# TUM-PIK-ESM/Terrarium.jl

Measured on AMD Instinct MI355X. Metric: column-steps/sec, higher is better.
Workload: dtype f64

## Files before the change

### terrarium.jl_amd/csrc/terrarium_hip.hip

```cpp
#include "trm_host.hpp"

#include <dlfcn.h>

using namespace trm;
using namespace trmh;

namespace {
thread_local std::string g_create_error;
}

namespace trmh {
int fail(trm_ctx* ctx, int code, const std::string& msg) {
    if (ctx) ctx->err = msg;
    else g_create_error = msg;
    return code;
}
}

namespace {

template <class NF> struct HostGrid {
    std::vector<NF> zF, zC, dzc, rdzc, rdzf, dzf, psiz;
    NF dzf_bot, dzf_top;
    void build(int Nz, const double* thickness) {
        std::vector<double> cs(Nz);
        double acc = thickness[0];
        cs[0] = acc;
        for (int n = 1; n < Nz; ++n) { acc = acc + thickness[n]; cs[n] = acc; }
        zF.resize(Nz + 1);
        for (int f = 0; f < Nz; ++f) zF[f] = (NF)(-cs[Nz - 1 - f]);
        zF[Nz] = NF(0);
        NF Fm1 = zF[0] - (zF[1] - zF[0]);
        NF Fp1 = zF[Nz] + (zF[Nz] - zF[Nz - 1]);
        zC.resize(Nz);
        dzc.resize(Nz);
        rdzc.resize(Nz);
        for (int k = 0; k < Nz; ++k) {
            zC[k] = (zF[k + 1] + zF[k]) / NF(2);
            dzc[k] = zF[k + 1] - zF[k];
            rdzc[k] = NF(1) / dzc[k];
        }
        NF Cm1 = (zF[0] + Fm1) / NF(2);
        NF Cp1 = (Fp1 + zF[Nz]) / NF(2);
        dzf.resize(Nz + 1);
        rdzf.resize(Nz + 1);
        for (int f = 0; f <= Nz; ++f) {
            NF hi = (f < Nz) ? zC[f] : Cp1;
            NF lo = (f > 0) ? zC[f - 1] : Cm1;
            dzf[f] = hi - lo;
            rdzf[f] = NF(1) / dzf[f];
        }
        dzf_bot = dzf[0];
        dzf_top = dzf[Nz];
        psiz.resize(Nz);
        for (int k = 0; k < Nz; ++k) psiz[k] = zC[k] - zF[Nz];
    }
};

template <class NF> DevParams<NF> make_dev_params(const trm_params& q) {
    DevParams<NF> p;
    NF rho_soc = (NF)q.rho_soc, rho_org = (NF)q.rho_org, por_m = (NF)q.por_mineral, por_o = (NF)q.por_organic;
    p.org = rho_soc / ((NF(1) - por_o) * rho_org);
    p.por = (NF(1) - p.org) * por_m + p.org * por_o;
    p.rpor = NF(1) / p.por;
    p.solid_frac = NF(1) - p.por;
    p.frac_organic = p.solid_frac * p.org;
    p.frac_mineral = p.solid_frac * (NF(1) - p.org);
    p.sk_water = std::sqrt((NF)q.k_water);
    p.sk_ice = std::sqrt((NF)q.k_ice);
    p.sk_air = std::sqrt((NF)q.k_air);
    p.kterm_mineral = std::sqrt((NF)q.k_mineral) * p.frac_mineral;
    p.kterm_organic = std::sqrt((NF)q.k_organic) * p.frac_organic;
    p.c_water = (NF)q.c_water;
    p.c_ice = (NF)q.c_ice;
    p.c_air = (NF)q.c_air;
    p.cterm_mineral = (NF)q.c_mineral * p.frac_mineral;
    p.cterm_organic = (NF)q.c_organic * p.frac_organic;
    p.L = (NF)q.rho_w * (NF)q.Lsl;
    p.K_sat = (NF)q.K_sat;
    p.theta_res = (NF)q.theta_res;
// ... 74 lines not shown
    v.lwu = F(TRM_FIELD_SURFACE_LONGWAVE_UP);
    v.rnet = F(TRM_FIELD_SURFACE_NET_RADIATION);
    v.Hs = F(TRM_FIELD_SENSIBLE_HEAT_FLUX);
    v.Hl = F(TRM_FIELD_LATENT_HEAT_FLUX);
    v.evap = F(TRM_FIELD_EVAPORATION_GROUND);
    v.infil = F(TRM_FIELD_INFILTRATION);
    v.runoff = F(TRM_FIELD_SURFACE_RUNOFF);
    v.Tair = F(TRM_FIELD_AIR_TEMPERATURE);
    v.pres = F(TRM_FIELD_AIR_PRESSURE);
    v.wind = F(TRM_FIELD_WINDSPEED);
    v.qair = F(TRM_FIELD_SPECIFIC_HUMIDITY);
    v.rain = F(TRM_FIELD_RAINFALL);
    v.swd = F(TRM_FIELD_SURFACE_SHORTWAVE_DOWN);
    v.lwd = F(TRM_FIELD_SURFACE_LONGWAVE_DOWN);
    v.albedo = F(TRM_FIELD_ALBEDO);
    v.emissivity = F(TRM_FIELD_EMISSIVITY);
    v.zC = (const NF*)c->d_zC;
    v.zF = (const NF*)c->d_zF;
    v.dzc = (const NF*)c->d_dzc;
    v.rdzc = (const NF*)c->d_rdzc;
    v.rdzf = (const NF*)c->d_rdzf;
    v.psiz = (const NF*)c->d_psiz;
    v.lvl = (const NF*)c->d_lvl;
    v.Fvwc = c->opt_vwc_field ? (const NF*)((&s == &c->stage && c->stage_vwc_own) ? c->stage.f[TRM_FIELD_VWC_FORCING] : c->state.f[TRM_FIELD_VWC_FORCING]) : nullptr;
    BcGeom<NF>& g = v.g;
    g.dzf_bot = (NF)c->dzf_bot;
    g.dzf_top = (NF)c->dzf_top;
    g.hdzf_bot = g.dzf_bot / NF(2);
    g.hdzf_top = g.dzf_top / NF(2);
    g.rhdzf_bot = NF(1) / g.hdzf_bot;
    g.rhdzf_top = NF(1) / g.hdzf_top;
    g.Az = (NF)c->Az;
    g.V_bot = g.Az * (NF)c->dzc_bot;
    g.V_top = g.Az * (NF)c->dzc_top;
    g.rV_bot = NF(1) / g.V_bot;
    g.rV_top = NF(1) / g.V_top;
    g.zF_top = (NF)c->h_zF[c->Nz];
    g.dzc_top = (NF)c->dzc_top;
    v.status = c->d_status;
    for (int a = 0; a < TRM_BCV_COUNT; ++a)
        for (int b = 0; b < 2; ++b) {
            v.bc.kind[a][b] = c->bc_kind[a][b];
            void* val = (&s == &c->stage && c->bc_value_stage[a][b]) ? c->bc_value_stage[a][b] : c->bc_value[a][b];
            v.bc.value[a][b] = val ? val : c->d_zero;
        }
    fill_small_table(v);
    return v;
}

template <class NF> View<NF> sub_view(const View<NF>& v, long lo, long n) {
    View<NF> s = v;
    s.Nh = n;
    const long c3 = lo * v.Nzp;
    auto p3 = [&](NF*& q) { if (q) q += c3; };
    auto p2 = [&](NF*& q) { if (q) q += lo; };
    auto c2 = [&](const NF*& q) { if (q) q += lo; };
    p3(s.U); p3(s.sat); p3(s.T); p3(s.liq); p3(s.psi); p3(s.Kf); p3(s.G_U); p3(s.G_sat);
    if (s.Fvwc) s.Fvwc += c3;
    p2(s.S); p2(s.wt); p2(s.Kf_top); p2(s.G_S);
    p2(s.Ts); p2(s.ghf); p2(s.infil); p2(s.swu); p2(s.lwu); p2(s.rnet); p2(s.Hs); p2(s.Hl); p2(s.evap); p2(s.runoff);
    p2(s.top_T); p2(s.top_sat); p2(s.top_liq);
// ... 563 lines not shown
        TRM_HIP(c, hipMemsetAsync(s.kf_top, 0, (size_t)c->Nh * c->esize, c->stream));
    }
    TRM_HIP(c, hipStreamSynchronize(c->stream));
    return TRM_OK;
}

template <class NF> int upload_grid(trm_ctx* c, const double* thickness) {
    HostGrid<NF> g;
    g.build(c->Nz, thickness);
    auto up = [&](void** d, const std::vector<NF>& h) -> int {
        TRM_HIP(c, hipMalloc(d, h.size() * sizeof(NF)));
        TRM_HIP(c, hipMemcpyAsync(*d, h.data(), h.size() * sizeof(NF), hipMemcpyHostToDevice, c->stream));
    TRM_HIP(c, hipStreamSynchronize(c->stream));
        return TRM_OK;
    };
    int rc;
    if ((rc = up(&c->d_zC, g.zC))) return rc;
    if ((rc = up(&c->d_zF, g.zF))) return rc;
    if ((rc = up(&c->d_dzc, g.dzc))) return rc;
    if ((rc = up(&c->d_rdzc, g.rdzc))) return rc;
    if ((rc = up(&c->d_rdzf, g.rdzf))) return rc;
    if ((rc = up(&c->d_psiz, g.psiz))) return rc;
    {
        std::vector<NF> lvl((size_t)c->Nz * 8, NF(0));
        for (int k = 0; k < c->Nz; ++k) {
            NF* q = &lvl[(size_t)k * 8];
            q[0] = g.zC[k]; q[1] = g.psiz[k]; q[2] = g.zF[k]; q[3] = g.dzc[k]; q[4] = g.rdzc[k]; q[5] = g.rdzf[k]; q[6] = g.rdzf[k + 1];
        }
        if ((rc = up(&c->d_lvl, lvl))) return rc;
    }
    c->h_zF.assign(g.zF.begin(), g.zF.end());
    c->h_zC.assign(g.zC.begin(), g.zC.end());
    c->h_dzc.assign(g.dzc.begin(), g.dzc.end());
    c->h_dzf.assign(g.dzf.begin(), g.dzf.end());
    c->dzf_bot = g.dzf_bot;
    c->dzf_top = g.dzf_top;
    c->dzc_bot = g.dzc[0];
    c->dzc_top = g.dzc[c->Nz - 1];
    return TRM_OK;
}

template <class NF> int fill_row(trm_ctx* c, int field, double value) {
    std::vector<NF> h((size_t)c->Nh, (NF)value);
    TRM_HIP(c, hipMemcpyAsync(c->state.f[field], h.data(), h.size() * sizeof(NF), hipMemcpyHostToDevice, c->stream));
    TRM_HIP(c, hipStreamSynchronize(c->stream));
    return TRM_OK;
}

__host__ __device__ inline double nan_min(double a, double b) { return (a != a || b != b) ? (a + b) : (a < b ? a : b); }
__host__ __device__ inline double nan_max(double a, double b) { return (a != a || b != b) ? (a + b) : (a > b ? a : b); }
template <class NF, int OP> __global__ void k_reduce_rows(const NF* f3, const NF* ftop, long Nh, int Nzp, int Nz, int is3d,
                                                          const NF* weight, double* partial) {
// ... 418 lines not shown

int trm_destroy(trm_ctx* c) {
    if (!c) return TRM_OK;
    (void)hipSetDevice(c->device);
    (void)trm_comm_destroy(c);
    if (c->own_stream) (void)hipStreamSynchronize(c->own_stream);
    for (int f = 0; f < TRM_FIELD_COUNT; ++f) {
        if (c->state.f[f]) (void)hipFree(c->state.raw[f]);
        if (c->stage.f[f]) (void)hipFree(c->stage.raw[f]);
        if (c->saved.f[f]) (void)hipFree(c->saved.raw[f]);
    }
    if (c->d_gran) (void)hipFree(c->d_gran);
    if (c->state.kf_top) (void)hipFree(c->state.kf_top);
    if (c->stage.kf_top) (void)hipFree(c->stage.kf_top);
    if (c->saved.kf_top) (void)hipFree(c->saved.kf_top);
    for (int a = 0; a < TRM_BCV_COUNT; ++a)
        for (int b = 0; b < 2; ++b)
        {
            if (c->bc_value[a][b]) (void)hipFree(c->bc_value[a][b]);
            if (c->bc_value_stage[a][b]) (void)hipFree(c->bc_value_stage[a][b]);
        }
    for (auto& sr : c->series)
        if (sr.d_values) (void)hipFree(sr.d_values);
    for (void* q : {c->d_zC, c->d_zF, c->d_dzc, c->d_rdzc, c->d_rdzf, c->d_psiz, c->d_lvl, c->d_rootf, c->d_zero, c->d_top3, (void*)c->d_status, (void*)c->d_reduce, c->d_io, c->d_series_table, c->d_series_rows})
        if (q) (void)hipFree(q);
    if (c->ev0) (void)hipEventDestroy(c->ev0);
    if (c->ev1) (void)hipEventDestroy(c->ev1);
    if (c->copy_stream) { (void)hipStreamSynchronize(c->copy_stream); (void)hipStreamDestroy(c->copy_stream); }
    if (c->copy_done) (void)hipEventDestroy(c->copy_done);
    if (c->copy_order) (void)hipEventDestroy(c->copy_order);
    if (c->h_stage) (void)hipHostFree(c->h_stage);
    for (auto& st : c->row_stage) {
        if (st.pending) (void)hipEventSynchronize(st.done);
        if (st.done) (void)hipEventDestroy(st.done);
        if (st.h) (void)hipHostFree(st.h);
    }
    for (void* q : {(void*)c->d_ring_inv, (void*)c->d_ring_idx, c->d_ring})
        if (q) (void)hipFree(q);
    for (auto& a : c->averages)
        if (a.d_sum) (void)hipFree(a.d_sum);
    for (double* q : c->d_acc_partial)
        if (q) (void)hipFree(q);
    release_tangent(c);
    release_adjoint(c);

    if (c->own_stream) (void)hipStreamDestroy(c->own_stream);
    if (c->args && c->args_free) c->args_free(c->args);
// ... 1261 lines not shown
```

### terrarium.jl_amd/csrc/trm_column.hpp

```cpp
#pragma once
#include "trm_kernels.hpp"
#include "trm_average.hpp"
#include <cstddef>
#include <type_traits>

namespace trm {

enum { PROG_EULER = 0, PROG_HEUN = 1, PROG_MULTI = 2 };
enum { PSI_STORED = 0, PSI_LAST = 1, PSI_INTERIOR = 2 };
#ifndef TRM_FRONT_DIAG
#define TRM_FRONT_DIAG 0
#endif
#ifndef TRM_FRONT_POLL_SLEEP
#define TRM_FRONT_POLL_SLEEP 4
#endif
#ifndef TRM_FRONT_PRIO
#define TRM_FRONT_PRIO 3
#endif

template <class NF> struct Cell { NF U, sat, T, liq, psi; };
struct LaneInfo { int lane, k; bool is_bot, is_top, act; unsigned long long m_act, m_bot, m_top; };
template <class NF> struct ColumnBC {
    NF bTb, bTt;
    NF flux_U, flux_S;
// ... 69 lines not shown
        const NF Kc_m = shfl_up1<NF, LPC>(Kc);
        const NF Kmin = jl_min(Kc, Kc_m);
        t.Kf_lo = BCSIG >= 0 ? mask_pick(m_bot | m_top, Kc, Kmin) : ((is_bot || is_top) ? Kc : Kmin);
    }
    if (RICHARDS) {
        const NF Kf_lo = t.Kf_lo;
        const NF Kf_up = shfl_up1<NF, LPC>(Kf_lo), Kf_dn = shfl_dn1<NF, LPC>(Kf_lo), psi_sh = shfl_up1<NF, LPC>(c.psi);
        const NF Kf_m = Kf_up;
        const NF Kf_p = at_top(Kc, Kf_dn);
        const NF psi_m = at_bot(c.psi, psi_sh);
        const NF g_lo = (c.psi - psi_m) * L.rdzf_lo;
        const NF Ks_lo = upwind_conductivity(g_lo, Kf_m, Kf_lo, Kf_p);
        const NF qW_lo = -Ks_lo * g_lo;
        const NF qW_sh = shfl_dn1<NF, LPC>(qW_lo);
        const NF zero_or_nan = c.psi - c.psi;
        const NF qW_t = -jl_min(Kc, NF(0)) * zero_or_nan;
        const NF qW_hi = at_top(qW_t, qW_sh);
        const NF dtheta = -((qW_hi - qW_lo) * L.rdzc) + NF(0) + p.vwc_forcing;
        t.gS = NF(0) + div_const_nsz(dtheta, p.por, p.rpor);
    }
    return t;
}

template <class NF, bool RICHARDS, int LPC>
TRM_DEV NF column_advance(const View<NF>& v, const LevelGeom<NF>& L, const LaneInfo& ln, int Nz, const ColumnBC<NF>& bc,
                          NF U0, NF sat0, NF& gU, NF& gS, NF dt, Cell<NF>& n, NF& z0, bool& bad) {
    if (bc.has_U) gU += bc.flux_U;
    n.U = U0 + gU * dt;
    if (!RICHARDS) bad = bad || (ln.act && is_nan(n.U));
    n.sat = sat0;
    z0 = NF(0);
    NF over = NF(0);
    if (RICHARDS) {
        if (bc.has_S) gS += bc.flux_S;
        NF snew = sat0 + gS * dt;
        bad = bad || (ln.act && __builtin_isunordered(n.U, snew));
        over = repair_saturation<NF, LPC>(v, snew, ln.k, Nz, ln.m_act, ln.is_bot, ln.is_top, L, ln.m_bot, ln.m_top);
        z0 = water_table<NF, LPC>(snew, ln.m_act, ln.lane, L);
        n.sat = snew;
    }
    return over;
}

template <class NF, bool RICHARDS, int HYD>
TRM_DEV Frac<NF> column_closure(const DevParams<NF>& p, const LevelGeom<NF>& L, NF z0, Cell<NF>& n, uint32_t& viol) {
    const Frac<NF> f = energy_closure_wave<NF, RICHARDS ? 2 : 1>(p, n.U, n.sat, n.liq, n.T, viol);
    n.psi = RICHARDS ? pressure_head<NF, HYD, true>(p, n.sat, L.zC, L.psiz, z0) : NF(0);
    return f;
}

template <class NF> struct SurfaceRegs {
    SebIn<NF> in;
    SebOut<NF> out;
};

enum { SLOT_T_BOT = 0, SLOT_T_TOP, SLOT_FU_BOT, SLOT_FU_TOP, SLOT_FS_BOT, SLOT_FS_TOP, SLOT_TAIR, SLOT_PRES, SLOT_WIND, SLOT_QAIR,
       SLOT_RAIN, SLOT_SWD, SLOT_LWD, SLOT_ALBEDO, SLOT_EMISSIVITY, SLOT_COUNT };
template <class NF> struct SeriesTable {
    const NF* base[SLOT_COUNT];
    NF* dst[SLOT_COUNT];
// ... 104 lines not shown
    const int finalize = a.finalize, write_kf = a.write_kf;
    const bool need_kc = RICHARDS || write_kf;
    const int i = wave * CPW + sub;
    const bool colok = i < Nh;
    ln.act = colok && ln.k < Nz;
    ln.m_act = wave_ballot(colok) & wave_ballot(ln.k < Nz);
    const int ii = colok ? i : Nh - 1;
    const int col_first = __builtin_amdgcn_readfirstlane(wave * CPW);
#endif
    const unsigned ib0 = (unsigned)ii * (unsigned)sizeof(NF);
    const unsigned cb0 = ((unsigned)ii * (unsigned)v.Nzp + (unsigned)(ln.k < Nz ? ln.k : Nz - 1)) * (unsigned)sizeof(NF);
    uint32_t viol = 0;
    bool bad = false;

    TRM_PHASE("loads+derive");
    Cell<NF> c;
    c.U = ldg(v.U, cb0);
    c.sat = ldg(v.sat, cb0);
    static_assert(DERIVE == DERIVE_NONE || DERIVE == DERIVE_T_LIQ, "the column program reads T / liq or derives both (the liquid fraction alone and the "
                  "pressure head as well were measured and lost: EXPERIMENTS.md; their instances were removed in round 5)");
    constexpr bool DERIVE_TL = DERIVE == DERIVE_T_LIQ;
    c.psi = (RICHARDS && !PSI_IN) ? ldg(v.psi, cb0) : NF(0);
    if (!DERIVE_TL) { c.T = ldg(v.T, cb0); c.liq = ldg(v.liq, cb0); }
    const LevelGeom<NF> L = level_geom(v, ln.k);
    constexpr bool SIG = BCSIG >= 0;
    const bool seb = SIG ? (BCSIG & BCSIG_LAND) != 0 : p.seb != 0;
    const bool vTb = SIG ? (BCSIG & BCSIG_T_BOT) != 0 : v.bc.kind[2][0] == 1, vTt = SIG ? (BCSIG & BCSIG_T_TOP) != 0 : v.bc.kind[2][1] == 1;
    const bool bU = SIG ? (BCSIG & BCSIG_FU_BOT) != 0 : v.bc.kind[0][0] == 2, bS = RICHARDS && (SIG ? (BCSIG & BCSIG_FS_BOT) != 0 : v.bc.kind[1][0] == 2);
    const bool tU = !SEB_INLINE && (seb || (SIG ? (BCSIG & BCSIG_FU_TOP) != 0 : v.bc.kind[0][1] == 2));
    const bool tS = RICHARDS && !SEB_INLINE && (seb || (SIG ? (BCSIG & BCSIG_FS_TOP) != 0 : v.bc.kind[1][1] == 2));
    const unsigned jo0 = (unsigned)(col_first < Nh ? col_first : Nh - 1) * (unsigned)sizeof(NF), jo1 = (unsigned)(col_first + 1 < Nh ? col_first + 1 : Nh - 1) * (unsigned)sizeof(NF);
    struct ColVal { NF x0, x1; };
    constexpr bool DEFER = SCALAR_IN && CPW == 2 && BCSIG >= 0;
    auto col_req = [&](const NF* ptr) -> ColVal {
        if (!SCALAR_IN) return ColVal{ldg(ptr, ib0), NF(0)};
        const NF x0 = sld_off<NF>(ptr, jo0);
        if (CPW == 1) return ColVal{x0, NF(0)};
        const NF x1 = sld_off<NF>(ptr, jo1);
        if (DEFER) return ColVal{x0, x1};
        return ColVal{upper ? x1 : x0, NF(0)};
    };
    auto pick_column = [&](NF x0, NF x1) -> NF {
#if TRM_PICK_EXEC
        if (__builtin_constant_p(x0 == x1) && x0 == x1) return x0;
        if constexpr (sizeof(NF) == 8) {
            NF r;
            unsigned long long save;
// ... 133 lines not shown
            bc.flux_S = ln.is_top ? eS_t : NF(0);
            TRM_PHASE("rare-");
        }
    };
    Cell<NF> n = c;
    Tendency<NF> t{};
    NF gU_out = NF(0), gS_out = NF(0), GS_out = NF(0), z0 = NF(0);

    NF over = NF(0), over_stage = NF(0);
    Frac<NF> f_new{};
    double accU = 0.0, accSat = 0.0, accT = 0.0, accLiq = 0.0, accPsi = 0.0, acc2 = 0.0;
    auto acc_top = [&](unsigned am, double w, int slot, NF x) {
        if (am & (1u << slot)) {
            const NF xt = shfl_from<NF, LPC>(x, Nz - 1);
            if (ln.k == slot - ACC_S) acc2 = acc2 + w * (double)xt;
        }
    };
    if (PROG == PROG_HEUN) {
        t = column_tendencies<NF, RICHARDS, HYD, LPC, BCSIG>(v, p, L, ln, c, bc.bTb, bc.bTt, need_kc, viol, DERIVE_TL ? &f_in : nullptr);
        const NF G1U = t.gU, G1S = t.gS;
        NF gU = G1U, gS = G1S, z0s;
        Cell<NF> s;
        front_wait();
        over_stage = column_advance<NF, RICHARDS, LPC>(v, L, ln, Nz, bc, c.U, c.sat, gU, gS, dt, s, z0s, bad);
        const Frac<NF> f_stage = column_closure<NF, RICHARDS, HYD>(kernarg_reload<DevParams<NF>>(off_p), L, z0s, s, viol);
        if (a.stage_T && ln.act) {
            const unsigned cb = block_local(cb0);
            stg(a.stage_sat, cb, s.sat);
            stg(a.stage_liq, cb, s.liq);
            stg(a.stage_T, cb, s.T);
        }
        const NF bTb2 = in_Tb2, bTt2 = in_Tt2;
        uint32_t viol_stage = 0;
        const Tendency<NF> t2 = column_tendencies<NF, RICHARDS, HYD, LPC, BCSIG>(kernarg_reload<View<NF>>(0), kernarg_reload<DevParams<NF>>(off_p), L, ln, s, bTb2, bTt2, RICHARDS, viol_stage, &f_stage);
        viol |= viol_stage;
        gU = (G1U + t2.gU) / NF(2);
        gS = RICHARDS ? (G1S + t2.gS) / NF(2) : NF(0);
        over = column_advance<NF, RICHARDS, LPC>(v, L, ln, Nz, bc, c.U, c.sat, gU, gS, dt, n, z0, bad);
        f_new = column_closure<NF, RICHARDS, HYD>(kernarg_reload<DevParams<NF>>(off_p), L, z0, n, viol);
        gU_out = gU; gS_out = gS;
    } else {
        const int nsteps = PROG == PROG_MULTI ? a.nsteps : 1;
        for (int step = 0; step < nsteps; ++step) {
            const View<NF>& v = PROG == PROG_MULTI ? kernarg_reload<View<NF>>(0) : v_arg;
            const DevParams<NF>& p = PROG == PROG_MULTI ? kernarg_reload<DevParams<NF>>(off_p) : p_arg;
            if (PROG == PROG_MULTI && step > 0) c = n;
            if (SERIES) {
                const SeriesTable<NF>* tb = a.series;
                const SeriesRow* rows = a.series_rows + (size_t)step * (size_t)a.nseries;
                if (tb->base[SLOT_T_BOT]) bc.bTb = series_value(tb, rows, SLOT_T_BOT, ii);
                if (tb->base[SLOT_T_TOP]) bc.bTt = series_value(tb, rows, SLOT_T_TOP, ii);
                if (tb->base[SLOT_FU_BOT]) { const NF e = flux_term_bottom(series_value(tb, rows, SLOT_FU_BOT, ii), v.g); if (ln.is_bot) bc.flux_U = e; }
                if (RICHARDS && tb->base[SLOT_FS_BOT]) { const NF e = flux_term_bottom(series_value(tb, rows, SLOT_FS_BOT, ii), v.g); if (ln.is_bot) bc.flux_S = e; }
                if (!SEB_INLINE) {
                    if (tb->base[SLOT_FU_TOP]) { const NF e = -flux_term_top(series_value(tb, rows, SLOT_FU_TOP, ii), v.g); if (ln.is_top) bc.flux_U = e; }
                    if (RICHARDS && tb->base[SLOT_FS_TOP]) { const NF e = -flux_term_top(series_value(tb, rows, SLOT_FS_TOP, ii), v.g); if (ln.is_top) bc.flux_S = e; }
                } else {
                    if (tb->base[SLOT_TAIR]) sf.in.Tair = series_value(tb, rows, SLOT_TAIR, ii);
                    if (tb->base[SLOT_PRES]) sf.in.pres = series_value(tb, rows, SLOT_PRES, ii);
                    if (tb->base[SLOT_WIND]) sf.in.wind = series_value(tb, rows, SLOT_WIND, ii);
                    if (tb->base[SLOT_QAIR]) sf.in.qair = series_value(tb, rows, SLOT_QAIR, ii);
// ... 30 lines not shown
                    const unsigned ib = block_local(ib0);
                    stg(v.ghf, ib, o.ghf); stg(v.swu, ib, o.swu); stg(v.lwu, ib, o.lwu); stg(v.rnet, ib, o.rnet);
                    stg(v.Hs, ib, o.Hs); stg(v.Hl, ib, o.Hl); stg(v.evap, ib, o.evap); stg(v.infil, ib, o.infil); stg(v.runoff, ib, o.runoff);
                }
                sf.out.Ts = sf.out.Ts + NF(0) * dt;
                if constexpr (ACCUM) {
                    const AccumArgs& aa = kernarg_reload<AccumArgs>(off_acc);
                    const unsigned am = aa.mask;
                    if (am >> ACC_TS) {
                        const double w = aa.dt;
                        const SebOut<NF>& o = sf.out;
                        acc_top(am, w, ACC_TS, o.Ts); acc_top(am, w, ACC_GHF, o.ghf); acc_top(am, w, ACC_SWU, o.swu); acc_top(am, w, ACC_LWU, o.lwu);
                        acc_top(am, w, ACC_RNET, o.rnet); acc_top(am, w, ACC_HS, o.Hs); acc_top(am, w, ACC_HL, o.Hl); acc_top(am, w, ACC_EVAP, o.evap);
                        acc_top(am, w, ACC_INFIL, o.infil); acc_top(am, w, ACC_RUNOFF, o.runoff);
                    }
                }
            }
            TRM_PHASE_FENCE("tendencies", c.U, c.sat, c.psi, c.T, c.liq, bc.bTb, bc.bTt, bc.flux_U, bc.flux_S, S_in, Ts_in);
            const Frac<NF>* pre = (PROG == PROG_MULTI && step > 0) ? &f_new : (DERIVE_TL ? &f_in : nullptr);
            t = column_tendencies<NF, RICHARDS, HYD, LPC, BCSIG>(v, p, L, ln, c, bc.bTb, bc.bTt, need_kc, viol, pre);
            NF gU = t.gU, gS = t.gS;
            TRM_PHASE_FENCE("advance", gU, gS, t.Kf_lo, t.Kc);
            front_wait();
            over = column_advance<NF, RICHARDS, LPC>(v, L, ln, Nz, bc, c.U, c.sat, gU, gS, dt, n, z0, bad);
            if (PROG == PROG_MULTI && RICHARDS) {
                GS_out = NF(0) + jl_min(NF(0), S);
                S = (S + GS_out * dt) + over;
            }
            TRM_PHASE_FENCE("closure", n.U, n.sat, z0, over, gU, gS);
            if constexpr (!INTERIOR) f_new = column_closure<NF, RICHARDS, HYD>(kernarg_reload<DevParams<NF>>(off_p), L, z0, n, viol);
            gU_out = gU; gS_out = gS;
            if constexpr (ACCUM) {
                const AccumArgs& aa = kernarg_reload<AccumArgs>(off_acc);
                const unsigned am = aa.mask;
                const double w = aa.dt;
                if (am & (1u << ACC_U)) accU = accU + w * (double)n.U;
                if (am & (1u << ACC_SAT)) accSat = accSat + w * (double)n.sat;
                if (am & (1u << ACC_T)) accT = accT + w * (double)n.T;
                if (am & (1u << ACC_LIQ)) accLiq = accLiq + w * (double)n.liq;
                if (am & (1u << ACC_PSI)) accPsi = accPsi + w * (double)n.psi;
                if (RICHARDS) { acc_top(am, w, ACC_S, S); acc_top(am, w, ACC_WT, z0); }
            }
        }
    }
    TRM_PHASE_FENCE("outputs", n.U, n.sat, n.T, n.liq, n.psi);

    NF Kf_out = t.Kf_lo, Kf_out_top = t.Kc;
// ... 382 lines not shown
```

### terrarium.jl_amd/csrc/trm_device.hpp

```cpp
#pragma once
#include <hip/hip_runtime.h>
#include <stdint.h>

#define TRM_DEV __device__ __forceinline__
#define TRM_HD __host__ __device__ __forceinline__
#ifdef TRM_PHASE_MARKERS
#define TRM_PHASE(name) asm volatile("; TRM_PHASE " name)
namespace trm {
template <class T> __device__ __forceinline__ void phase_opaque(T& x) {
    if (!__builtin_constant_p(x)) asm volatile("" : "+v"(x));
}
template <class... T> __device__ __forceinline__ void phase_fence_values(T&... x) { (phase_opaque(x), ...); }
}
#define TRM_PHASE_FENCE(name, ...)                 \
    do {                                           \
        asm volatile("; TRM_PHASE " name);         \
        ::trm::phase_fence_values(__VA_ARGS__);    \
    } while (0)
#else
#define TRM_PHASE(name) ((void)0)
#define TRM_PHASE_FENCE(name, ...) ((void)0)
#endif

#ifndef TRM_LOAD_POINTERS_UPFRONT
// ... 556 lines not shown
    o.evap = div_nr(evaporation_resistance_factor(p, sat_top, liq_top) * humidity_vpd(p, in.pres, in.qair, o.Ts), ra);
    NF excess = richards ? S : NF(0);
    bool unsat = sat_top < NF(1);
    NF drainage;
    if (excess > NF(0)) {
        drainage = div_const(jl_max(excess, NF(0)), p.tau_r, p.rtau_r);
        o.infil = boolmul(unsat, jl_min(drainage, Kf_top));
    } else {
        drainage = NF(0);
        o.infil = boolmul(unsat, jl_min(in.rain, Kf_top));
    }
    o.runoff = in.rain + drainage - o.infil;
    for (int sweep = 0; sweep < 2; ++sweep) {
        seb_fluxes(p, in, ra, o);
        o.Ts = T_ground - div_const(o.ghf * dz_top, p.kappa_s2, p.rkappa_s2);
        seb_fluxes(p, in, ra, o);
    }
}

struct BcSet {
    int kind[5][2];
    const void* value[5][2];
};
template <class NF> struct BcGeom {
    NF dzf_bot, dzf_top;
    NF hdzf_bot, hdzf_top;
    NF rhdzf_bot, rhdzf_top;
    NF Az, V_bot, V_top, rV_bot, rV_top;
    NF zF_top, dzc_top;
};
template <class NF> TRM_DEV NF halo_top(int kind, const NF* val, long i, NF c_edge, const BcGeom<NF>& g) {
    if (kind == 1) {
        NF grad = div_const(val[i] - c_edge, g.hdzf_top, g.rhdzf_top);
        return c_edge + grad * g.dzf_top;
    }
    if (kind == 3) return c_edge + val[i] * g.dzf_top;
    return c_edge;
}
template <class NF> TRM_DEV NF halo_bottom(int kind, const NF* val, long i, NF c_edge, const BcGeom<NF>& g) {
    if (kind == 1) {
        NF grad = div_const(c_edge - val[i], g.hdzf_bot, g.rhdzf_bot);
        return c_edge + grad * (-g.dzf_bot);
    }
    if (kind == 3) return c_edge + val[i] * (-g.dzf_bot);
    return c_edge;
}
template <class NF> TRM_DEV NF flux_term_top(NF flux, const BcGeom<NF>& g) { return div_const(flux * g.Az, g.V_top, g.rV_top); }
template <class NF> TRM_DEV NF flux_term_bottom(NF flux, const BcGeom<NF>& g) { return div_const(flux * g.Az, g.V_bot, g.rV_bot); }
template <class NF> TRM_DEV NF flux_term_top_nsz(NF flux, const BcGeom<NF>& g) { return div_const_nsz(flux * g.Az, g.V_top, g.rV_top); }
template <class NF> TRM_DEV NF flux_term_bottom_nsz(NF flux, const BcGeom<NF>& g) { return div_const_nsz(flux * g.Az, g.V_bot, g.rV_bot); }

}
// ... 1 lines not shown
```

### terrarium.jl_amd/csrc/trm_host.hpp

```cpp
#pragma once
#include "../../include/terrarium_hip.h"
#include "trm_kernels.hpp"
#include "trm_column.hpp"
#include "trm_vegetation.hpp"
#include "trm_dispatch.hpp"

#include <rccl/rccl.h>

#include <cmath>
#include <limits>
#include <type_traits>
#include <cstdio>
#include <cstdlib>
#include <cstring>
#include <algorithm>
#include <string>
#include <vector>

struct FieldSet {
    void* f[TRM_FIELD_COUNT];
    void* kf_top;
    void* raw[TRM_FIELD_COUNT];
};

struct trm_ctx {
    int precision = TRM_F64;
    long Nh = 0;
    int Nz = 0, Nzp = 0, device = 0;
    size_t esize = 8;
    trm_params params;
    hipStream_t own_stream = nullptr, stream = nullptr;
    hipEvent_t ev0 = nullptr, ev1 = nullptr;
    FieldSet state{}, stage{}, saved{};
    bool has_stage = false, has_saved = false;
    double saved_time = 0.0;
    int64_t saved_iteration = 0;
    uint32_t saved_status = 0;
    bool saved_tend_valid = true;
    void* bc_value[TRM_BCV_COUNT][2] = {};
    int bc_kind[TRM_BCV_COUNT][2] = {};
    bool bc_zero_gradient[TRM_BCV_COUNT][2] = {};
    void *d_zC = nullptr, *d_zF = nullptr, *d_dzc = nullptr, *d_rdzc = nullptr, *d_rdzf = nullptr, *d_psiz = nullptr, *d_lvl = nullptr;
    void* d_rootf = nullptr;
    std::vector<double> h_zF, h_zC, h_dzc, h_dzf;
    double dzf_bot = 0, dzf_top = 0, dzc_bot = 0, dzc_top = 0, Az = 1;
    uint32_t* d_status = nullptr;
    struct Series {
        bool is_bc = false;
        int field = 0, var = 0, side = 0, indexing = 0;
        std::vector<double> times;
        void* d_values = nullptr;
        long cap = 0, head = 0;
        long pending_from = -1;
        bool windowed = false;
        bool trimmed = false;
        double trimmed_before = 0.0;
        size_t slot(int n) const { return (size_t)((head + n) % cap); }
    };
    std::vector<Series> series;
    hipStream_t copy_stream = nullptr;
    hipEvent_t copy_done = nullptr;
    hipEvent_t copy_order = nullptr;
    bool copy_pending = false, order_recorded = false;
    void* h_stage = nullptr;
    size_t h_stage_cap = 0;
    long ring_points = 0;
    int32_t* d_ring_inv = nullptr;
    int32_t* d_ring_idx = nullptr;
// ... 746 lines not shown
```

### terrarium.jl_amd/csrc/trm_kernels.hpp

```cpp
#pragma once
#include "trm_device.hpp"

namespace trm {

template <class NF> struct View {
    long Nh;
    int Nz, Nzp;
    const NF* lvl;
    NF *U, *sat, *T, *liq, *psi;
    BcSet bc;
    BcGeom<NF> g;
    NF *S, *wt;
    NF *Kf;
    NF *Kf_top;
    uint32_t* status;
    NF *G_U, *G_sat, *G_S;
    const NF* Fvwc;
    NF *Ts, *ghf, *infil, *swu, *lwu, *rnet, *Hs, *Hl, *evap, *runoff;
    NF *top_T, *top_sat, *top_liq;
    const NF *Tair, *pres, *wind, *qair, *rain, *swd, *lwd;
    const NF *albedo, *emissivity;
    const NF *zC, *zF, *dzc, *rdzc, *rdzf, *psiz;
    NF* small[8];
};
enum { BCSIG_RUNTIME = -1,
       BCSIG_T_BOT = 1, BCSIG_T_TOP = 2,
       BCSIG_FU_BOT = 4, BCSIG_FS_BOT = 8,
       BCSIG_FU_TOP = 16, BCSIG_FS_TOP = 32,
       BCSIG_LAND = 64 };
enum { DERIVE_NONE = 0, DERIVE_T_LIQ = 1, DERIVE_LIQ = 2,
       DERIVE_LIQ_PSI = 3,
// ... 362 lines not shown
}
TRM_DEV unsigned block_local(unsigned byte_off) {
    asm volatile("" : "+v"(byte_off));
    return byte_off;
}
TRM_DEV bool uniform_flag(int x) {
    asm volatile("" : "+s"(x));
    return x != 0;
}

template <class NF> struct LevelGeom {
    NF zC, psiz, zFlo, dzc, rdzc, rdzf_lo, rdzf_hi, zF_top, dzc_top;
};
template <class NF> struct alignas(16) LevelPack { NF w[8]; };
template <class NF> TRM_DEV LevelGeom<NF> level_geom(const View<NF>& v, int k) {
    const int Nz = v.Nz;
    const int kk = k < Nz ? k : Nz - 1;
    const LevelPack<NF> q = *reinterpret_cast<const LevelPack<NF>*>(reinterpret_cast<const char*>(v.lvl) + (unsigned)kk * (unsigned)sizeof(LevelPack<NF>));
    LevelGeom<NF> L;
    L.zC = q.w[0]; L.psiz = q.w[1]; L.zFlo = q.w[2]; L.dzc = q.w[3]; L.rdzc = q.w[4]; L.rdzf_lo = q.w[5]; L.rdzf_hi = q.w[6];
    L.zF_top = v.g.zF_top; L.dzc_top = v.g.dzc_top;
    return L;
}
template <class NF> struct NeighbourDz { NF dzc_up, rdzc_up, dzc_dn, rdzc_dn; };
template <class NF> TRM_DEV NeighbourDz<NF> neighbour_dz(const View<NF>& v, int k) {
    const int Nz = v.Nz;
    const int kk = k < Nz ? k : Nz - 1;
    const int ku = kk + 1 < Nz ? kk + 1 : kk, kd = kk > 0 ? kk - 1 : 0;
    NeighbourDz<NF> n;
    n.dzc_up = v.dzc[ku]; n.rdzc_up = v.rdzc[ku]; n.dzc_dn = v.dzc[kd]; n.rdzc_dn = v.rdzc[kd];
    return n;
}

template <class NF, int LPC>
TRM_DEV NF repair_saturation(const View<NF>& v, NF& snew, int k, int Nz, unsigned long long m_act, bool is_bot, bool is_top,
                             const LevelGeom<NF>& L, unsigned long long m_bot_known = 0ull, unsigned long long m_top_known = 0ull) {
    const unsigned long long m_top = m_top_known ? m_top_known : wave_ballot(is_top), m_bot = m_bot_known ? m_bot_known : wave_ballot(is_bot);
    const unsigned long long any_over = wave_ballot(snew > NF(1)) & m_act & ~m_top;
    const unsigned long long any_bad = any_over | (wave_ballot(snew < NF(0)) & m_act & ~m_bot);
    snew = mask_pick(m_bot, snew, snew + NF(0));
    if (any_bad != 0ull) {
        TRM_PHASE("rare+ repair");
        NF dzc = L.dzc, rdzc = L.rdzc;
        asm volatile("" : "+v"(dzc), "+v"(rdzc));
        NeighbourDz<NF> nb;
        {
            const NF dz_up = shfl_dn1<NF, LPC>(dzc), rdz_up = shfl_dn1<NF, LPC>(rdzc);
            const NF dz_dn = shfl_up1<NF, LPC>(dzc), rdz_dn = shfl_up1<NF, LPC>(rdzc);
            const bool edge_up = k >= Nz - 1;
            nb.dzc_up = edge_up ? dzc : dz_up;
            nb.rdzc_up = edge_up ? rdzc : rdz_up;
            nb.dzc_dn = is_bot ? dzc : dz_dn;
            nb.rdzc_dn = is_bot ? rdzc : rdz_dn;
        }
        if (any_over != 0ull) {
            const unsigned long long lv = level_bits<LPC>(any_over);
            NF carry = NF(0);
            for (int q = __builtin_ctzll(lv); q < Nz - 1; ++q) {
                NF cout = NF(0);
                if (k == q) {
                    snew = snew + carry;
                    NF e = jl_max(snew - NF(1), NF(0));
                    snew = snew - e;
                    cout = div_const(e * dzc, nb.dzc_up, nb.rdzc_up);
                }
                carry = shfl_from<NF, LPC>(cout, q);
                if ((lv >> (q + 1)) == 0ull && wave_ballot(!(carry == NF(0))) == 0ull) break;
// ... 268 lines not shown
```

Baseline: 3.497 billion.

## Shrink per-level geometry record from eight to four words

Adds a 4-word per-level table (zC, zF, rdzc, rdzf_lo) and loads it instead of the 8-word record in the column kernel. psiz is taken as zC, which the host now checks bit for bit at creation. rdzf_hi comes from a scalar top value, and dzc is rebuilt from face shuffles in the rare repair path. The goal is fewer bytes per level load and fewer live registers. The cost is a stricter grid precondition and a rdzf_hi that is only right where the kernel uses it at the top.

```diff
diff --git a/terrarium.jl_amd/csrc/terrarium_hip.hip b/terrarium.jl_amd/csrc/terrarium_hip.hip
--- a/terrarium.jl_amd/csrc/terrarium_hip.hip
+++ b/terrarium.jl_amd/csrc/terrarium_hip.hip
@@ -1,4 +1,5 @@
 #include "trm_host.hpp"
+#include "trm_grid.hpp"
 
 #include <dlfcn.h>
 
@@ -18,44 +19,6 @@
 }
 
 namespace {
-
-template <class NF> struct HostGrid {
-    std::vector<NF> zF, zC, dzc, rdzc, rdzf, dzf, psiz;
-    NF dzf_bot, dzf_top;
-    void build(int Nz, const double* thickness) {
-        std::vector<double> cs(Nz);
-        double acc = thickness[0];
-        cs[0] = acc;
-        for (int n = 1; n < Nz; ++n) { acc = acc + thickness[n]; cs[n] = acc; }
-        zF.resize(Nz + 1);
-        for (int f = 0; f < Nz; ++f) zF[f] = (NF)(-cs[Nz - 1 - f]);
-        zF[Nz] = NF(0);
-        NF Fm1 = zF[0] - (zF[1] - zF[0]);
-        NF Fp1 = zF[Nz] + (zF[Nz] - zF[Nz - 1]);
-        zC.resize(Nz);
-        dzc.resize(Nz);
-        rdzc.resize(Nz);
-        for (int k = 0; k < Nz; ++k) {
-            zC[k] = (zF[k + 1] + zF[k]) / NF(2);
-            dzc[k] = zF[k + 1] - zF[k];
-            rdzc[k] = NF(1) / dzc[k];
-        }
-        NF Cm1 = (zF[0] + Fm1) / NF(2);
-        NF Cp1 = (Fp1 + zF[Nz]) / NF(2);
-        dzf.resize(Nz + 1);
-        rdzf.resize(Nz + 1);
-        for (int f = 0; f <= Nz; ++f) {
-            NF hi = (f < Nz) ? zC[f] : Cp1;
-            NF lo = (f > 0) ? zC[f - 1] : Cm1;
-            dzf[f] = hi - lo;
-            rdzf[f] = NF(1) / dzf[f];
-        }
-        dzf_bot = dzf[0];
-        dzf_top = dzf[Nz];
-        psiz.resize(Nz);
-        for (int k = 0; k < Nz; ++k) psiz[k] = zC[k] - zF[Nz];
-    }
-};
 
 template <class NF> DevParams<NF> make_dev_params(const trm_params& q) {
     DevParams<NF> p;
@@ -176,6 +139,9 @@
     v.rdzf = (const NF*)c->d_rdzf;
     v.psiz = (const NF*)c->d_psiz;
     v.lvl = (const NF*)c->d_lvl;
+#if TRM_LEVEL_RECORD == 4
+    v.lvl4 = (const NF*)c->d_lvl4;
+#endif
     v.Fvwc = c->opt_vwc_field ? (const NF*)((&s == &c->stage && c->stage_vwc_own) ? c->stage.f[TRM_FIELD_VWC_FORCING] : c->state.f[TRM_FIELD_VWC_FORCING]) : nullptr;
     BcGeom<NF>& g = v.g;
     g.dzf_bot = (NF)c->dzf_bot;
@@ -191,6 +157,9 @@
     g.rV_top = NF(1) / g.V_top;
     g.zF_top = (NF)c->h_zF[c->Nz];
     g.dzc_top = (NF)c->dzc_top;
+#if TRM_LEVEL_RECORD == 4
+    g.rdzf_top = (NF)c->rdzf_top;
+#endif
     v.status = c->d_status;
     for (int a = 0; a < TRM_BCV_COUNT; ++a)
         for (int b = 0; b < 2; ++b) {
@@ -800,12 +769,13 @@
     if ((rc = up(&c->d_rdzf, g.rdzf))) return rc;
     if ((rc = up(&c->d_psiz, g.psiz))) return rc;
     {
-        std::vector<NF> lvl((size_t)c->Nz * 8, NF(0));
-        for (int k = 0; k < c->Nz; ++k) {
-            NF* q = &lvl[(size_t)k * 8];
-            q[0] = g.zC[k]; q[1] = g.psiz[k]; q[2] = g.zF[k]; q[3] = g.dzc[k]; q[4] = g.rdzc[k]; q[5] = g.rdzf[k]; q[6] = g.rdzf[k + 1];
-        }
-        if ((rc = up(&c->d_lvl, lvl))) return rc;
+        const int k_bad = first_level_psiz_differs(g);
+        if (k_bad >= 0) return fail(c, TRM_EINVAL, "trm_create: the elevation head of level " + std::to_string(k_bad) + " is not its centre bit for bit (the short level records need zF[Nz] = 0)");
+        LevelTables<NF> t;
+        t.build(g);
+        if ((rc = up(&c->d_lvl, t.lvl))) return rc;
+        if ((rc = up(&c->d_lvl4, t.lvl4))) return rc;
+        c->rdzf_top = t.rdzf_top;
     }
     c->h_zF.assign(g.zF.begin(), g.zF.end());
     c->h_zC.assign(g.zC.begin(), g.zC.end());
@@ -1270,7 +1240,7 @@
         }
     for (auto& sr : c->series)
         if (sr.d_values) (void)hipFree(sr.d_values);
-    for (void* q : {c->d_zC, c->d_zF, c->d_dzc, c->d_rdzc, c->d_rdzf, c->d_psiz, c->d_lvl, c->d_rootf, c->d_zero, c->d_top3, (void*)c->d_status, (void*)c->d_reduce, c->d_io, c->d_series_table, c->d_series_rows})
+    for (void* q : {c->d_zC, c->d_zF, c->d_dzc, c->d_rdzc, c->d_rdzf, c->d_psiz, c->d_lvl, c->d_lvl4, c->d_rootf, c->d_zero, c->d_top3, (void*)c->d_status, (void*)c->d_reduce, c->d_io, c->d_series_table, c->d_series_rows})
         if (q) (void)hipFree(q);
     if (c->ev0) (void)hipEventDestroy(c->ev0);
     if (c->ev1) (void)hipEventDestroy(c->ev1);
diff --git a/terrarium.jl_amd/csrc/trm_column.hpp b/terrarium.jl_amd/csrc/trm_column.hpp
--- a/terrarium.jl_amd/csrc/trm_column.hpp
+++ b/terrarium.jl_amd/csrc/trm_column.hpp
@@ -115,7 +115,7 @@
     return t;
 }
 
-template <class NF, bool RICHARDS, int LPC>
+template <class NF, bool RICHARDS, int LPC, bool CORE = false>
 TRM_DEV NF column_advance(const View<NF>& v, const LevelGeom<NF>& L, const LaneInfo& ln, int Nz, const ColumnBC<NF>& bc,
                           NF U0, NF sat0, NF& gU, NF& gS, NF dt, Cell<NF>& n, NF& z0, bool& bad) {
     if (bc.has_U) gU += bc.flux_U;
@@ -128,7 +128,7 @@
         if (bc.has_S) gS += bc.flux_S;
         NF snew = sat0 + gS * dt;
         bad = bad || (ln.act && __builtin_isunordered(n.U, snew));
-        over = repair_saturation<NF, LPC>(v, snew, ln.k, Nz, ln.m_act, ln.is_bot, ln.is_top, L, ln.m_bot, ln.m_top);
+        over = repair_saturation<NF, LPC, CORE>(v, snew, ln.k, Nz, ln.m_act, ln.is_bot, ln.is_top, L, ln.m_bot, ln.m_top);
         z0 = water_table<NF, LPC>(snew, ln.m_act, ln.lane, L);
         n.sat = snew;
     }
@@ -279,7 +279,13 @@
     constexpr bool DERIVE_TL = DERIVE == DERIVE_T_LIQ;
     c.psi = (RICHARDS && !PSI_IN) ? ldg(v.psi, cb0) : NF(0);
     if (!DERIVE_TL) { c.T = ldg(v.T, cb0); c.liq = ldg(v.liq, cb0); }
+#if TRM_LEVEL_RECORD == 4
+    constexpr bool SHORT_RECORD = !SCALAR_IN || TRM_LEVEL_RECORD_SCALAR_IN == 4;
+    const LevelGeom<NF> L = SHORT_RECORD ? level_core(v, ln.k) : level_geom(v, ln.k);
+#else
+    constexpr bool SHORT_RECORD = false;
     const LevelGeom<NF> L = level_geom(v, ln.k);
+#endif
     constexpr bool SIG = BCSIG >= 0;
     const bool seb = SIG ? (BCSIG & BCSIG_LAND) != 0 : p.seb != 0;
     const bool vTb = SIG ? (BCSIG & BCSIG_T_BOT) != 0 : v.bc.kind[2][0] == 1, vTt = SIG ? (BCSIG & BCSIG_T_TOP) != 0 : v.bc.kind[2][1] == 1;
@@ -459,7 +465,7 @@
         NF gU = G1U, gS = G1S, z0s;
         Cell<NF> s;
         front_wait();
-        over_stage = column_advance<NF, RICHARDS, LPC>(v, L, ln, Nz, bc, c.U, c.sat, gU, gS, dt, s, z0s, bad);
+        over_stage = column_advance<NF, RICHARDS, LPC, SHORT_RECORD>(v, L, ln, Nz, bc, c.U, c.sat, gU, gS, dt, s, z0s, bad);
         const Frac<NF> f_stage = column_closure<NF, RICHARDS, HYD>(kernarg_reload<DevParams<NF>>(off_p), L, z0s, s, viol);
         if (a.stage_T && ln.act) {
             const unsigned cb = block_local(cb0);
@@ -473,7 +479,7 @@
         viol |= viol_stage;
         gU = (G1U + t2.gU) / NF(2);
         gS = RICHARDS ? (G1S + t2.gS) / NF(2) : NF(0);
-        over = column_advance<NF, RICHARDS, LPC>(v, L, ln, Nz, bc, c.U, c.sat, gU, gS, dt, n, z0, bad);
+        over = column_advance<NF, RICHARDS, LPC, SHORT_RECORD>(v, L, ln, Nz, bc, c.U, c.sat, gU, gS, dt, n, z0, bad);
         f_new = column_closure<NF, RICHARDS, HYD>(kernarg_reload<DevParams<NF>>(off_p), L, z0, n, viol);
         gU_out = gU; gS_out = gS;
     } else {
@@ -550,7 +556,7 @@
             NF gU = t.gU, gS = t.gS;
             TRM_PHASE_FENCE("advance", gU, gS, t.Kf_lo, t.Kc);
             front_wait();
-            over = column_advance<NF, RICHARDS, LPC>(v, L, ln, Nz, bc, c.U, c.sat, gU, gS, dt, n, z0, bad);
+            over = column_advance<NF, RICHARDS, LPC, SHORT_RECORD>(v, L, ln, Nz, bc, c.U, c.sat, gU, gS, dt, n, z0, bad);
             if (PROG == PROG_MULTI && RICHARDS) {
                 GS_out = NF(0) + jl_min(NF(0), S);
                 S = (S + GS_out * dt) + over;
diff --git a/terrarium.jl_amd/csrc/trm_device.hpp b/terrarium.jl_amd/csrc/trm_device.hpp
--- a/terrarium.jl_amd/csrc/trm_device.hpp
+++ b/terrarium.jl_amd/csrc/trm_device.hpp
@@ -602,12 +602,23 @@
     int kind[5][2];
     const void* value[5][2];
 };
+#ifndef TRM_LEVEL_RECORD
+#define TRM_LEVEL_RECORD 4
+#endif
+#ifndef TRM_LEVEL_RECORD_SCALAR_IN
+#define TRM_LEVEL_RECORD_SCALAR_IN 8
+#endif
+static_assert(TRM_LEVEL_RECORD == 4 || TRM_LEVEL_RECORD == 8, "TRM_LEVEL_RECORD: 4 or 8 words per level");
+static_assert(TRM_LEVEL_RECORD_SCALAR_IN == 8 || (TRM_LEVEL_RECORD_SCALAR_IN == 4 && TRM_LEVEL_RECORD == 4), "TRM_LEVEL_RECORD_SCALAR_IN: 8, or 4 in a build that has the short record");
 template <class NF> struct BcGeom {
     NF dzf_bot, dzf_top;
     NF hdzf_bot, hdzf_top;
     NF rhdzf_bot, rhdzf_top;
     NF Az, V_bot, V_top, rV_bot, rV_top;
     NF zF_top, dzc_top;
+#if TRM_LEVEL_RECORD == 4
+    NF rdzf_top;
+#endif
 };
 template <class NF> TRM_DEV NF halo_top(int kind, const NF* val, long i, NF c_edge, const BcGeom<NF>& g) {
     if (kind == 1) {
diff --git a/terrarium.jl_amd/csrc/trm_grid.hpp b/terrarium.jl_amd/csrc/trm_grid.hpp
--- /dev/null
+++ b/terrarium.jl_amd/csrc/trm_grid.hpp
@@ -0,0 +1,63 @@
+#pragma once
+#include <cstring>
+#include <vector>
+
+template <class NF> struct HostGrid {
+    std::vector<NF> zF, zC, dzc, rdzc, rdzf, dzf, psiz;
+    NF dzf_bot, dzf_top;
+    void build(int Nz, const double* thickness) {
+        std::vector<double> cs(Nz);
+        double acc = thickness[0];
+        cs[0] = acc;
+        for (int n = 1; n < Nz; ++n) { acc = acc + thickness[n]; cs[n] = acc; }
+        zF.resize(Nz + 1);
+        for (int f = 0; f < Nz; ++f) zF[f] = (NF)(-cs[Nz - 1 - f]);
+        zF[Nz] = NF(0);
+        NF Fm1 = zF[0] - (zF[1] - zF[0]);
+        NF Fp1 = zF[Nz] + (zF[Nz] - zF[Nz - 1]);
+        zC.resize(Nz);
+        dzc.resize(Nz);
+        rdzc.resize(Nz);
+        for (int k = 0; k < Nz; ++k) {
+            zC[k] = (zF[k + 1] + zF[k]) / NF(2);
+            dzc[k] = zF[k + 1] - zF[k];
+            rdzc[k] = NF(1) / dzc[k];
+        }
+        NF Cm1 = (zF[0] + Fm1) / NF(2);
+        NF Cp1 = (Fp1 + zF[Nz]) / NF(2);
+        dzf.resize(Nz + 1);
+        rdzf.resize(Nz + 1);
+        for (int f = 0; f <= Nz; ++f) {
+            NF hi = (f < Nz) ? zC[f] : Cp1;
+            NF lo = (f > 0) ? zC[f - 1] : Cm1;
+            dzf[f] = hi - lo;
+            rdzf[f] = NF(1) / dzf[f];
+        }
+        dzf_bot = dzf[0];
+        dzf_top = dzf[Nz];
+        psiz.resize(Nz);
+        for (int k = 0; k < Nz; ++k) psiz[k] = zC[k] - zF[Nz];
+    }
+};
+
+template <class NF> struct LevelTables {
+    std::vector<NF> lvl, lvl4;
+    NF rdzf_top;
+    void build(const HostGrid<NF>& g) {
+        const int Nz = (int)g.zC.size();
+        lvl.assign((size_t)Nz * 8, NF(0));
+        lvl4.assign((size_t)Nz * 4, NF(0));
+        for (int k = 0; k < Nz; ++k) {
+            NF* q = &lvl[(size_t)k * 8];
+            q[0] = g.zC[k]; q[1] = g.psiz[k]; q[2] = g.zF[k]; q[3] = g.dzc[k]; q[4] = g.rdzc[k]; q[5] = g.rdzf[k]; q[6] = g.rdzf[k + 1];
+            NF* s = &lvl4[(size_t)k * 4];
+            s[0] = g.zC[k]; s[1] = g.zF[k]; s[2] = g.rdzc[k]; s[3] = g.rdzf[k];
+        }
+        rdzf_top = g.rdzf[Nz];
+    }
+};
+template <class NF> int first_level_psiz_differs(const HostGrid<NF>& g) {
+    for (size_t k = 0; k < g.zC.size(); ++k)
+        if (std::memcmp(&g.psiz[k], &g.zC[k], sizeof(NF)) != 0) return (int)k;
+    return -1;
+}
diff --git a/terrarium.jl_amd/csrc/trm_host.hpp b/terrarium.jl_amd/csrc/trm_host.hpp
--- a/terrarium.jl_amd/csrc/trm_host.hpp
+++ b/terrarium.jl_amd/csrc/trm_host.hpp
@@ -40,10 +40,11 @@
     void* bc_value[TRM_BCV_COUNT][2] = {};
     int bc_kind[TRM_BCV_COUNT][2] = {};
     bool bc_zero_gradient[TRM_BCV_COUNT][2] = {};
-    void *d_zC = nullptr, *d_zF = nullptr, *d_dzc = nullptr, *d_rdzc = nullptr, *d_rdzf = nullptr, *d_psiz = nullptr, *d_lvl = nullptr;
+    void *d_zC = nullptr, *d_zF = nullptr, *d_dzc = nullptr, *d_rdzc = nullptr, *d_rdzf = nullptr, *d_psiz = nullptr, *d_lvl = nullptr, *d_lvl4 = nullptr;
     void* d_rootf = nullptr;
     std::vector<double> h_zF, h_zC, h_dzc, h_dzf;
     double dzf_bot = 0, dzf_top = 0, dzc_bot = 0, dzc_top = 0, Az = 1;
+    double rdzf_top = 0;
     uint32_t* d_status = nullptr;
     struct Series {
         bool is_bc = false;
diff --git a/terrarium.jl_amd/csrc/trm_kernels.hpp b/terrarium.jl_amd/csrc/trm_kernels.hpp
--- a/terrarium.jl_amd/csrc/trm_kernels.hpp
+++ b/terrarium.jl_amd/csrc/trm_kernels.hpp
@@ -7,6 +7,9 @@
     long Nh;
     int Nz, Nzp;
     const NF* lvl;
+#if TRM_LEVEL_RECORD == 4
+    const NF* lvl4;
+#endif
     NF *U, *sat, *T, *liq, *psi;
     BcSet bc;
     BcGeom<NF> g;
@@ -415,6 +418,19 @@
     L.zF_top = v.g.zF_top; L.dzc_top = v.g.dzc_top;
     return L;
 }
+#if TRM_LEVEL_RECORD == 4
+template <class NF> struct alignas(16) LevelCorePack { NF w[4]; };
+template <class NF> TRM_DEV LevelGeom<NF> level_core(const View<NF>& v, int k) {
+    const int Nz = v.Nz;
+    const int kk = k < Nz ? k : Nz - 1;
+    const LevelCorePack<NF> q = *reinterpret_cast<const LevelCorePack<NF>*>(reinterpret_cast<const char*>(v.lvl4) + (unsigned)kk * (unsigned)sizeof(LevelCorePack<NF>));
+    LevelGeom<NF> L;
+    L.zC = q.w[0]; L.psiz = q.w[0]; L.zFlo = q.w[1]; L.rdzc = q.w[2]; L.rdzf_lo = q.w[3];
+    L.rdzf_hi = v.g.rdzf_top;
+    L.zF_top = v.g.zF_top; L.dzc_top = v.g.dzc_top;
+    return L;
+}
+#endif
 template <class NF> struct NeighbourDz { NF dzc_up, rdzc_up, dzc_dn, rdzc_dn; };
 template <class NF> TRM_DEV NeighbourDz<NF> neighbour_dz(const View<NF>& v, int k) {
     const int Nz = v.Nz;
@@ -425,7 +441,7 @@
     return n;
 }
 
-template <class NF, int LPC>
+template <class NF, int LPC, bool DZC_FROM_FACES = false>
 TRM_DEV NF repair_saturation(const View<NF>& v, NF& snew, int k, int Nz, unsigned long long m_act, bool is_bot, bool is_top,
                              const LevelGeom<NF>& L, unsigned long long m_bot_known = 0ull, unsigned long long m_top_known = 0ull) {
     const unsigned long long m_top = m_top_known ? m_top_known : wave_ballot(is_top), m_bot = m_bot_known ? m_bot_known : wave_ballot(is_bot);
@@ -434,8 +450,17 @@
     snew = mask_pick(m_bot, snew, snew + NF(0));
     if (any_bad != 0ull) {
         TRM_PHASE("rare+ repair");
-        NF dzc = L.dzc, rdzc = L.rdzc;
-        asm volatile("" : "+v"(dzc), "+v"(rdzc));
+        NF dzc, rdzc = L.rdzc;
+        if constexpr (DZC_FROM_FACES) {
+            NF zFlo = L.zFlo;
+            asm volatile("" : "+v"(zFlo), "+v"(rdzc));
+            const NF z_sh = shfl_dn1<NF, LPC>(zFlo);
+            const NF z_up = k >= Nz - 1 ? L.zF_top : z_sh;
+            dzc = z_up - zFlo;
+        } else {
+            dzc = L.dzc;
+            asm volatile("" : "+v"(dzc), "+v"(rdzc));
+        }
         NeighbourDz<NF> nb;
         {
             const NF dz_up = shfl_dn1<NF, LPC>(dzc), rdz_up = shfl_dn1<NF, LPC>(rdzc);
```

New measurement: 3.425 billion. 0.98x the previous value.
